# CrawlScript/tf_geometric

Measured on NVIDIA H100. Metric: edges/sec GCN+GAT fwd on 2.4M-node/123M-edge synthetic; %HBM roofline, higher is better.
Workload: dtype f32

## Files before the change

### include/tfgk.h

```cpp
#ifndef TFGK_H_
#define TFGK_H_

#include <stddef.h>
#include <stdint.h>

#ifdef __cplusplus
extern "C" {
#endif

#define TFGK_ABI_VERSION 7

enum tfgk_status {
    TFGK_OK = 0,
    TFGK_ERR_INVALID_ARGUMENT = 1,
    TFGK_ERR_CUDA = 2,
    TFGK_ERR_WORKSPACE = 3,
    TFGK_ERR_UNSUPPORTED = 4,
    TFGK_ERR_INDEX_OUT_OF_RANGE = 5
};

enum tfgk_reduce { TFGK_REDUCE_SUM = 0, TFGK_REDUCE_MEAN = 1, TFGK_REDUCE_MAX = 2 };
enum tfgk_act { TFGK_ACT_NONE = 0, TFGK_ACT_RELU = 1 };
enum tfgk_deg_power { TFGK_POW_INV_SQRT = 0, TFGK_POW_INV = 1 };
enum tfgk_heads_mode { TFGK_HEADS_SPLIT = 0, TFGK_HEADS_BROADCAST = 1, TFGK_HEADS_REDUCE = 2 };
// ... 50 lines not shown
int tfgk_permute_f32(const float *src, const int32_t *perm, int64_t E, int32_t width, float *dst, void *stream);
int tfgk_unpermute_f32(const float *src, const int32_t *perm, int64_t E, int32_t width, float *dst, void *stream);


int tfgk_csr_rowsum_f32(const int64_t *rowptr, const float *w_csr, int32_t N, float *out, void *stream);
int tfgk_deg_inv_f32(const float *deg, int32_t N, int power, float *out, void *stream);
int tfgk_scale_edges_f32(const int32_t *row, const int32_t *col, const float *w, int64_t E,
                         const float *dl, const float *dr, float *out, void *stream);


int tfgk_spmm_f32(const int64_t *rowptr, const int32_t *col, const float *w,
                  const float *h, int64_t ldh, int32_t n_dst, int32_t D, int reduce,
                  float alpha, const float *addend, int64_t ld_addend, float beta,
                  const float *bias, int act,
                  float *out, int64_t ldo, const tfgk_plan *plan, void *stream);
int tfgk_spmm_bf16(const int64_t *rowptr, const int32_t *col, const float *w,
                   const uint16_t *h, int64_t ldh, int32_t n_dst, int32_t D, int reduce,
                   float alpha, const float *addend, int64_t ld_addend, float beta,
                   const float *bias, int act,
                   float *out, int64_t ldo, const tfgk_plan *plan, void *stream);
int tfgk_spmm_bf16_dual(const int64_t *rowptr, const int32_t *col, const float *w,
                        const uint16_t *h, int64_t ldh, int32_t n_dst, int32_t D, int reduce,
                        float alpha, const float *addend, int64_t ld_addend, float beta,
                        const float *bias, int act,
                        float *out, int64_t ldo, uint16_t *out_bf16, int64_t ldob,
                        const tfgk_plan *plan, void *stream);

int tfgk_spmm_fp8(const int64_t *rowptr, const int32_t *col, const float *w,
                  const uint8_t *h, int64_t ldh, const int8_t *h_exp, int32_t n_dst, int32_t D, int reduce,
                  float alpha, const float *addend, int64_t ld_addend, float beta,
// ... 234 lines not shown
```

### tf_geometric_b200/_ffi.py

```python
import ctypes
import os
import threading

_LIB_PATH = os.path.join(os.path.dirname(os.path.abspath(__file__)), "lib", "libtfgk.so")
_lock = threading.Lock()
_lib = None

ABI_VERSION = 7

OK = 0
ERR_INVALID_ARGUMENT, ERR_CUDA, ERR_WORKSPACE, ERR_UNSUPPORTED, ERR_INDEX_OUT_OF_RANGE = 1, 2, 3, 4, 5
REDUCE_SUM, REDUCE_MEAN, REDUCE_MAX = 0, 1, 2
ACT_NONE, ACT_RELU = 0, 1
POW_INV_SQRT, POW_INV = 0, 1
HEADS_SPLIT, HEADS_BROADCAST, HEADS_REDUCE = 0, 1, 2
FLAG_ALL, FLAG_UPPER, FLAG_MAPPED = 0, 1, 2
BERNOULLI_NONE, BERNOULLI_DROPOUT, BERNOULLI_KEEP = 0, 1, 2
SAMPLE_NO_PADDING, SAMPLE_PADDING, SAMPLE_HEAD = 0, 1, 2
NEG_UPPER, NEG_START = 0, 1
PAD_ROW_MAJOR, PAD_STEP_MAJOR = 0, 1
SPGEMM_GRAD_LEFT, SPGEMM_GRAD_RIGHT = 0, 1
DTYPE_F32, DTYPE_BF16, DTYPE_FP8_E4M3 = 0, 1, 2

_i32, _i64, _f32, _int = ctypes.c_int32, ctypes.c_int64, ctypes.c_float, ctypes.c_int
# ... 11 lines not shown
    "tfgk_edge_unique_workspace_bytes": [_i64, _i32, ctypes.POINTER(_size)],
    "tfgk_edge_unique": [_ptr, _ptr, _i64, _i32, _ptr, _ptr, ctypes.POINTER(_i32), _ptr, _size, _ptr],
    "tfgk_directed_workspace_bytes": [_i64, ctypes.POINTER(_size)],
    "tfgk_directed_edges": [_ptr, _i64, _i64, _ptr, _i64, _ptr, ctypes.POINTER(_i32), _ptr, _size, _ptr],
    "tfgk_plan_capacity": [_i64, _i32, _i32, _i32, _i32, ctypes.POINTER(_i64), ctypes.POINTER(_i64)],
    "tfgk_plan_workspace_bytes": [_i32, ctypes.POINTER(_size)],
    "tfgk_plan_build": [_ptr, _i32, _i32, _i32, _i32, _ptr, _ptr, _ptr, _ptr, _ptr, _ptr, _ptr, _ptr, _i64, _i64,
                        ctypes.POINTER(_i32), _ptr, _size, _ptr],
    "tfgk_permute_f32": [_ptr, _ptr, _i64, _i32, _ptr, _ptr],
    "tfgk_unpermute_f32": [_ptr, _ptr, _i64, _i32, _ptr, _ptr],
    "tfgk_csr_rowsum_f32": [_ptr, _ptr, _i32, _ptr, _ptr],
    "tfgk_deg_inv_f32": [_ptr, _i32, _int, _ptr, _ptr],
    "tfgk_scale_edges_f32": [_ptr, _ptr, _ptr, _i64, _ptr, _ptr, _ptr, _ptr],
    "tfgk_spmm_f32": [_ptr, _ptr, _ptr, _ptr, _i64, _i32, _i32, _int, _f32, _ptr, _i64, _f32, _ptr, _int, _ptr, _i64,
                      _ptr, _ptr],
    "tfgk_spmm_bf16": [_ptr, _ptr, _ptr, _ptr, _i64, _i32, _i32, _int, _f32, _ptr, _i64, _f32, _ptr, _int, _ptr, _i64,
                       _ptr, _ptr],
    "tfgk_spmm_bf16_dual": [_ptr, _ptr, _ptr, _ptr, _i64, _i32, _i32, _int, _f32, _ptr, _i64, _f32, _ptr, _int, _ptr,
                            _i64, _ptr, _i64, _ptr, _ptr],
    "tfgk_spmm_fp8": [_ptr, _ptr, _ptr, _ptr, _i64, _ptr, _i32, _i32, _int, _f32, _ptr, _i64, _f32, _ptr, _int, _ptr,
                      _i64, _ptr, _ptr],
    "tfgk_segment_softmax_f32": [_ptr, _ptr, _i32, _i32, _ptr, _ptr],
    "tfgk_gat_fused_f32": [_ptr, _ptr, _ptr, _i64, _ptr, _i64, _ptr, _i64, _i32, _i32, _i32, _i32, _f32, _int, _ptr,
                           _int, _ptr, _int, _ptr, _i64, _ptr, _ptr],
    "tfgk_gat_fused_bf16": [_ptr, _ptr, _ptr, _i64, _ptr, _i64, _ptr, _i64, _i32, _i32, _i32, _i32, _f32, _int, _ptr,
                            _int, _ptr, _int, _ptr, _i64, _ptr, _ptr],
    "tfgk_gat_fused_fp8": [_ptr, _ptr, _ptr, _i64, _ptr, _i64, _ptr, _i32, _i32, _i32, _f32, _ptr, _int, _ptr, _i64, _ptr,
                           _ptr],
    "tfgk_gat_pack_keys_f32": [_ptr, _i64, _i32, _i32, _ptr, _i64, _ptr, _ptr],
    "tfgk_gat_fused_packed_f32": [_ptr, _ptr, _ptr, _i64, _ptr, _i64, _ptr, _i32, _i32, _i32, _f32, _ptr, _int, _ptr, _i64,
# ... 210 lines not shown
```

### tf_geometric_b200/csrc/spmm.cu

```cuda
#include "common.cuh"
#include <cuda_bf16.h>

namespace tfgk {

template <int VEC> struct Vec;
template <> struct Vec<4> { using T = float4; };
template <> struct Vec<1> { using T = float; };

template <int VEC>
__device__ __forceinline__ void load_vec(const float *p, float (&v)[VEC]) {
    if constexpr (VEC == 4) {
        const float4 t = __ldg(reinterpret_cast<const float4 *>(p));
        v[0] = t.x; v[1] = t.y; v[2] = t.z; v[3] = t.w;
    } else {
        v[0] = __ldg(p);
    }
}

template <int VEC>
__device__ __forceinline__ void load_vec(const uint16_t *p, float (&v)[VEC]) {
    static_assert(VEC == 1, "bf16 rows take the scalar path");
    v[0] = bf16_to_f32(__ldg(p));
}

// ... 32 lines not shown
    const float *bias;
    int act;
    float *out;
    int64_t ldo;
    uint16_t *outb;
    int64_t ldob;
    int32_t d_store;
    bool io4;
    int32_t n_tasks;
    const int32_t *task_row, *task_nrows;
    const int64_t *task_e0, *task_e1;
    const int32_t *task_slot;
    int32_t n_hubs;
    const int32_t *hub_row, *hub_slot0, *hub_nslots;
    float *scratch;
};

template <typename T> __device__ __forceinline__ const T *rows_of(const SpmmParams &p);
template <> __device__ __forceinline__ const float *rows_of<float>(const SpmmParams &p) { return p.h; }
template <> __device__ __forceinline__ const uint16_t *rows_of<uint16_t>(const SpmmParams &p) { return p.hb; }
template <> __device__ __forceinline__ const uint8_t *rows_of<uint8_t>(const SpmmParams &p) { return p.h8; }

template <int N>
__device__ __forceinline__ void epilogue_dual(const SpmmParams &p, int64_t r, int c, const float (&acc)[N], float cnt) {
    if (c >= p.d_store) return;
    float ad[N], bs[N], o[N];
    if constexpr (N == 4) {
        if (p.io4) {
            if (p.addend) load_vec<4>(p.addend + r * p.ld_addend + c, ad);
            if (p.bias) load_vec<4>(p.bias + c, bs);
// ... 316 lines not shown
        }
        if ((g + S) % RPC == 0) {
            const int dead = (g + S) / RPC - 1;
            if (dead & 1) load_chunk(dead + 2, cb, wnb); else load_chunk(dead + 2, ca, wna);
        }
    }
    if (slot >= 0) {
#pragma unroll
        for (int k = 0; k < NC; ++k)
            if (cok[k]) store_vec<4>(p.scratch + (int64_t)slot * p.D + coff[k], acc[k]);
        return;
    }
    while (r < r1) finalize_row();
}

__device__ __forceinline__ void tma_row(uint32_t dst, const void *src, uint32_t bytes, uint32_t bar) {
    asm volatile("cp.async.bulk.shared::cluster.global.mbarrier::complete_tx::bytes [%0], [%1], %2, [%3];"
                 ::"r"(dst), "l"(src), "r"(bytes), "r"(bar) : "memory");
}

__device__ __forceinline__ void mbar_wait_parity(uint32_t bar, uint32_t parity) {
    uint32_t done = 0;
    for (uint32_t spin = 0; !done; ++spin) {
        asm volatile(
            "{\n\t.reg .pred p;\n\t"
            "mbarrier.try_wait.parity.shared::cta.b64 p, [%1], %2;\n\t"
            "selp.u32 %0, 1, 0, p;\n\t}"
            : "=r"(done) : "r"(bar), "r"(parity) : "memory");
        if (spin > (1u << 28)) __trap();
    }
}

template <bool IS_MAX, int S, typename T, bool DUAL = false>
__global__ void __launch_bounds__(kAsyncWarps * 32) spmm_tma4_kernel(const SpmmParams p, uint32_t row_bytes) {
    constexpr int U = 4, RPC = 32 / U;
    constexpr bool FP8 = sizeof(T) == 1;
    static_assert(S <= 2 * RPC, "weight look-ahead registers would be overwritten before they are consumed");
    extern __shared__ __align__(128) uint8_t g4_ring[];
    const int lane = threadIdx.x & 31, warp = threadIdx.x >> 5;
    const uint32_t stage_bytes = (U * row_bytes + 127u) & ~127u;
    uint8_t *my_ring = g4_ring + (size_t)warp * S * stage_bytes;
    const uint32_t ring_addr = (uint32_t)__cvta_generic_to_shared(my_ring);
    uint64_t *bars = reinterpret_cast<uint64_t *>(g4_ring + (size_t)kAsyncWarps * S * stage_bytes) + warp * S;
    uint16_t *sexp = reinterpret_cast<uint16_t *>(g4_ring + (size_t)kAsyncWarps * S * (stage_bytes + 8)) + warp * S * U;
    const uint32_t bar0 = (uint32_t)__cvta_generic_to_shared(bars);
    if (lane == 0) {
#pragma unroll
        for (int i = 0; i < S; ++i) asm volatile("mbarrier.init.shared::cta.b64 [%0], 1;" ::"r"(bar0 + 8 * i));
        asm volatile("fence.mbarrier_init.release.cluster;" ::: "memory");
    }
    __syncwarp();
    const int64_t task = (int64_t)blockIdx.x * kAsyncWarps + warp;
    int64_t r0, r1, e_begin, e_stop;
    int slot = -1;
    if (p.task_row != nullptr) {
        if (task >= p.n_tasks) return;
        r0 = p.task_row[task];
        r1 = r0 + p.task_nrows[task];
        e_begin = p.task_e0[task];
        e_stop = p.task_e1[task];
        slot = p.task_slot[task];
    } else {
        r0 = task * kAsyncRows;
        if (r0 >= p.n_dst) return;
        r1 = min((int64_t)p.n_dst, r0 + kAsyncRows);
        e_begin = p.rowptr[r0];
        e_stop = p.rowptr[r1];
// ... 6 lines not shown
    constexpr int NCX = 2;
    int coff[NCX];
    bool cok[NCX];
    float acc[NCX][4];
#pragma unroll
    for (int k = 0; k < NCX; ++k) {
        coff[k] = (lane + 32 * k) * 4;
        cok[k] = coff[k] < p.D;
#pragma unroll
        for (int x = 0; x < 4; ++x) acc[k][x] = IS_MAX ? -FLT_MAX : 0.0f;
    }
    int64_t r = r0;
    int row_end = slot >= 0 ? 0x7fffffff : (int)(__shfl_sync(0xffffffffu, rp_hi, 0) - e_begin);
    const bool is_mean = p.reduce == TFGK_REDUCE_MEAN;

    auto finalize_row = [&]() {
        const int64_t row_start = __shfl_sync(0xffffffffu, rp_lo, (int)(r - r0));
        const int deg = (int)(row_end + e_begin - row_start);
        const float cnt = (float)max(deg, 1);
#pragma unroll
        for (int k = 0; k < NCX; ++k) {
            if (DUAL && cok[k]) {
                epilogue_dual<4>(p, r, coff[k], acc[k], cnt);
#pragma unroll
                for (int x = 0; x < 4; ++x) acc[k][x] = IS_MAX ? -FLT_MAX : 0.0f;
            } else if (cok[k]) {
                float ad[4], bs[4], o[4];
                if (p.addend) load_vec<4>(p.addend + r * p.ld_addend + coff[k], ad);
                if (p.bias) load_vec<4>(p.bias + coff[k], bs);
#pragma unroll
                for (int x = 0; x < 4; ++x) {
                    float a = acc[k][x];
                    if (is_mean) a = __fdiv_rn(a, cnt);
                    if (p.addend) a = __fadd_rn(__fmul_rn(a, p.alpha), __fmul_rn(ad[x], p.beta));
                    else if (p.alpha != 1.0f) a = __fmul_rn(a, p.alpha);
                    if (p.bias) a = __fadd_rn(a, bs[x]);
                    o[x] = apply_act(a, p.act);
                    acc[k][x] = IS_MAX ? -FLT_MAX : 0.0f;
                }
                store_vec<4>(p.out + r * p.ldo + coff[k], o);
            }
        }
        ++r;
        if (r < r1) row_end = (int)(__shfl_sync(0xffffffffu, rp_hi, (int)(r - r0)) - e_begin);
    };
    auto load_chunk = [&](int c, int &ci, float &wi) {
        const int e = c * 32 + lane;
        ci = 0;
        wi = 1.0f;
        if (e < n_edges) {
            ci = ld_stream_i32(p.col + e_begin + e);
            if (weighted) wi = ld_stream_f32(p.w + e_begin + e);
        }
    };
    uint32_t xpend = 0;
    int xslot = -1;
    auto issue = [&](int g, int ci) {
        if constexpr (FP8) {
// ... 69 lines not shown
        if ((g + 1) % RPC == 0) {
            if (cc & 1) wb = wnb; else wa = wna;
        }
        if ((g + S) % RPC == 0) {
            const int dead = (g + S) / RPC - 1;
            if (dead & 1) load_chunk(dead + 2, cb, wnb); else load_chunk(dead + 2, ca, wna);
        }
    }
    if (slot >= 0) {
#pragma unroll
        for (int k = 0; k < NCX; ++k)
            if (cok[k]) store_vec<4>(p.scratch + (int64_t)slot * p.D + coff[k], acc[k]);
        return;
    }
    while (r < r1) finalize_row();
}

template <bool IS_MAX, bool DUAL = false>
__global__ void __launch_bounds__(256) spmm_hub_fixup_kernel(const SpmmParams p) {
    const int lane = threadIdx.x & 31;
    const int h = blockIdx.x * 8 + (threadIdx.x >> 5);
    if (h >= p.n_hubs) return;
    const int64_t r = p.hub_row[h];
    const int s0 = p.hub_slot0[h], ns = p.hub_nslots[h];
    const float cnt = (float)max((int)(p.rowptr[r + 1] - p.rowptr[r]), 1);
    for (int c = lane * 4; c < p.D; c += 128) {
        float acc[4] = {IS_MAX ? -FLT_MAX : 0.f, IS_MAX ? -FLT_MAX : 0.f, IS_MAX ? -FLT_MAX : 0.f, IS_MAX ? -FLT_MAX : 0.f};
        for (int s = 0; s < ns; ++s) {
            float v[4];
            load_vec<4>(p.scratch + (int64_t)(s0 + s) * p.D + c, v);
#pragma unroll
            for (int x = 0; x < 4; ++x) acc[x] = IS_MAX ? fmaxf(acc[x], v[x]) : __fadd_rn(acc[x], v[x]);
        }
        if constexpr (DUAL) {
            epilogue_dual<4>(p, r, c, acc, cnt);
            continue;
        }
        float ad[4], bs[4], o[4];
        if (p.addend) load_vec<4>(p.addend + r * p.ld_addend + c, ad);
        if (p.bias) load_vec<4>(p.bias + c, bs);
#pragma unroll
        for (int x = 0; x < 4; ++x) {
            float a = acc[x];
            if (p.reduce == TFGK_REDUCE_MEAN) a = __fdiv_rn(a, cnt);
            if (p.addend) a = __fadd_rn(__fmul_rn(a, p.alpha), __fmul_rn(ad[x], p.beta));
            else if (p.alpha != 1.0f) a = __fmul_rn(a, p.alpha);
            if (p.bias) a = __fadd_rn(a, bs[x]);
            o[x] = apply_act(a, p.act);
        }
        store_vec<4>(p.out + r * p.ldo + c, o);
    }
}

template <int NC, int U, int S, typename T = float, bool DUAL = false>
static int launch_spmm_async(const SpmmParams &p, cudaStream_t st) {
    const uint32_t row_bytes = (uint32_t)(p.D * sizeof(T));
    const size_t smem = (size_t)kAsyncWarps * S * U * row_bytes;
    if (smem > 200 * 1024) return TFGK_ERR_UNSUPPORTED;
    const int64_t n_tasks = p.task_row ? p.n_tasks : ceil_div64(p.n_dst, kAsyncRows);
    const unsigned blocks = (unsigned)ceil_div64(n_tasks, kAsyncWarps);
    if (p.reduce == TFGK_REDUCE_MAX) {
        TFGK_CUDA(ensure_dynamic_smem(spmm_async_kernel<NC, true, U, S, T, DUAL>, smem));
        spmm_async_kernel<NC, true, U, S, T, DUAL><<<blocks, kAsyncWarps * 32, smem, st>>>(p, row_bytes);
    } else {
        TFGK_CUDA(ensure_dynamic_smem(spmm_async_kernel<NC, false, U, S, T, DUAL>, smem));
        spmm_async_kernel<NC, false, U, S, T, DUAL><<<blocks, kAsyncWarps * 32, smem, st>>>(p, row_bytes);
    }
    TFGK_LAUNCH_CHECK();
    if (p.task_row && p.n_hubs > 0) {
        const unsigned fb = (unsigned)ceil_div64(p.n_hubs, 8);
        if (p.reduce == TFGK_REDUCE_MAX) spmm_hub_fixup_kernel<true, DUAL><<<fb, 256, 0, st>>>(p);
        else spmm_hub_fixup_kernel<false, DUAL><<<fb, 256, 0, st>>>(p);
        TFGK_LAUNCH_CHECK();
    }
    return TFGK_OK;
}

template <int S, typename T = float, bool DUAL = false>
static int launch_spmm_tma4(const SpmmParams &p, cudaStream_t st) {
    constexpr int kPer16 = 16 / (int)sizeof(T);
    const void *base = sizeof(T) == 4 ? (const void *)p.h : sizeof(T) == 2 ? (const void *)p.hb : (const void *)p.h8;
    if (p.D > 256 || p.D % kPer16 != 0 || p.ldh % kPer16 != 0 || !aligned16(base)) return TFGK_ERR_UNSUPPORTED;
    const uint32_t row_bytes = (uint32_t)(p.D * sizeof(T));
    const size_t stage_pitch = ((size_t)4 * row_bytes + 127) & ~(size_t)127;
    const size_t smem = (size_t)kAsyncWarps * S * stage_pitch + (size_t)kAsyncWarps * S * 8 +
                        (sizeof(T) == 1 ? (size_t)kAsyncWarps * S * 4 * sizeof(uint16_t) : 0);
    if (smem > 200 * 1024) return TFGK_ERR_UNSUPPORTED;
    const int64_t n_tasks = p.task_row ? p.n_tasks : ceil_div64(p.n_dst, kAsyncRows);
    const unsigned blocks = (unsigned)ceil_div64(n_tasks, kAsyncWarps);
    if (p.reduce == TFGK_REDUCE_MAX) {
        TFGK_CUDA(ensure_dynamic_smem(spmm_tma4_kernel<true, S, T, DUAL>, smem));
        spmm_tma4_kernel<true, S, T, DUAL><<<blocks, kAsyncWarps * 32, smem, st>>>(p, row_bytes);
    } else {
        TFGK_CUDA(ensure_dynamic_smem(spmm_tma4_kernel<false, S, T, DUAL>, smem));
        spmm_tma4_kernel<false, S, T, DUAL><<<blocks, kAsyncWarps * 32, smem, st>>>(p, row_bytes);
    }
    TFGK_LAUNCH_CHECK();
    if (p.task_row && p.n_hubs > 0) {
        const unsigned fb = (unsigned)ceil_div64(p.n_hubs, 8);
        if (p.reduce == TFGK_REDUCE_MAX) spmm_hub_fixup_kernel<true, DUAL><<<fb, 256, 0, st>>>(p);
        else spmm_hub_fixup_kernel<false, DUAL><<<fb, 256, 0, st>>>(p);
        TFGK_LAUNCH_CHECK();
    }
    return TFGK_OK;
}

template <typename T, bool DUAL = false>
static int dispatch_spmm_async(const SpmmParams &p, cudaStream_t st) {
    const int lanes = (p.D + 3) / 4;
    return lanes <= 32 ? launch_spmm_async<1, 4, 3, T, DUAL>(p, st)
         : lanes <= 64 ? launch_spmm_async<2, 4, 4, T, DUAL>(p, st)
         : lanes <= 96 ? launch_spmm_async<3, 4, 3, T, DUAL>(p, st)
                       : launch_spmm_async<4, 2, 4, T, DUAL>(p, st);
}

// ... 43 lines not shown
                              int reduce, float alpha, const float *addend, int64_t ld_addend, float beta,
                              const float *bias, int act, float *out, int64_t ldo, int c0, int width) {
    SpmmParams p;
    p.rowptr = rowptr; p.col = col; p.w = w;
    p.h = nullptr; p.hb = nullptr; p.ldh = ldh; p.n_dst = n_dst;
    p.h8 = nullptr; p.hexp = nullptr; p.n_grp = 0; p.grp0 = 0;
    p.D = width;
    p.reduce = reduce; p.alpha = alpha;
    p.addend = addend ? addend + c0 : nullptr; p.ld_addend = ld_addend; p.beta = beta;
    p.bias = bias ? bias + c0 : nullptr; p.act = act;
    p.out = out ? out + c0 : nullptr; p.ldo = ldo;
    p.outb = nullptr; p.ldob = 0; p.d_store = width; p.io4 = false;
    p.n_tasks = 0; p.task_row = nullptr; p.task_nrows = nullptr; p.task_e0 = nullptr; p.task_e1 = nullptr;
    p.task_slot = nullptr; p.n_hubs = 0; p.hub_row = nullptr; p.hub_slot0 = nullptr; p.hub_nslots = nullptr;
    p.scratch = nullptr;
    return p;
}

}

using namespace tfgk;

extern "C" int tfgk_spmm_f32(const int64_t *rowptr, const int32_t *col, const float *w,
                             const float *h, int64_t ldh, int32_t n_dst, int32_t D, int reduce,
                             float alpha, const float *addend, int64_t ld_addend, float beta,
                             const float *bias, int act,
                             float *out, int64_t ldo, const tfgk_plan *plan, void *stream) {
    bool nothing_to_do = true;
    const int vrc = spmm_validate(rowptr, h, ldh, n_dst, D, reduce, addend, ld_addend, act, out, ldo, plan, &nothing_to_do);
    if (vrc != TFGK_OK || nothing_to_do) return vrc;
// ... 5 lines not shown
    for (int c0 = 0; c0 < D; c0 += cols_per_launch) {
        SpmmParams p = spmm_params(rowptr, col, w, ldh, n_dst, reduce, alpha, addend, ld_addend, beta, bias, act, out, ldo,
                                   c0, (D - c0 < cols_per_launch) ? D - c0 : cols_per_launch);
        p.h = h + c0;
        if (plan != nullptr && plan->n_tasks > 0 && vec4 && D >= 32 && D <= cols_per_launch) use_plan(p, plan);
        if (vec4 && p.D >= 32) {
            int rcr = launch_spmm_tma4<3>(p, as_stream(stream));
            if (rcr == TFGK_ERR_UNSUPPORTED) rcr = dispatch_spmm_async<float>(p, as_stream(stream));
            if (rcr != TFGK_ERR_UNSUPPORTED) { if (rcr != TFGK_OK) return rcr; continue; }
        }
        const int lanes = (p.D + vec - 1) / vec;
        const int rc = vec4 ? dispatch_spmm<4>(p, lanes, as_stream(stream)) : dispatch_spmm<1>(p, lanes, as_stream(stream));
        if (rc != TFGK_OK) return rc;
    }
    return TFGK_OK;
}

extern "C" int tfgk_spmm_bf16(const int64_t *rowptr, const int32_t *col, const float *w,
                              const uint16_t *h, int64_t ldh, int32_t n_dst, int32_t D, int reduce,
                              float alpha, const float *addend, int64_t ld_addend, float beta,
                              const float *bias, int act,
                              float *out, int64_t ldo, const tfgk_plan *plan, void *stream) {
    bool nothing_to_do = true;
    const int vrc = spmm_validate(rowptr, h, ldh, n_dst, D, reduce, addend, ld_addend, act, out, ldo, plan, &nothing_to_do);
    if (vrc != TFGK_OK || nothing_to_do) return vrc;

    const bool rows4 = (D % 4 == 0) && (ldh % 4 == 0) && aligned8(h) && (ldo % 4 == 0) && aligned16(out) &&
                       (!addend || ((ld_addend % 4 == 0) && aligned16(addend))) && (!bias || aligned16(bias));
    cudaStream_t st = as_stream(stream);
    if (rows4 && D >= 32 && D <= 512) {
// ... 107 lines not shown
```

### tf_geometric_b200/dist.py

```python
import os

import torch
import torch.distributed as dist

from . import ops
from .ops import CSR

ROW_ALIGN = 128


class RowPartition(object):

    def __init__(self, num_nodes, world_size, rank, align=1):
        self.num_nodes = int(num_nodes)
        self.world_size = int(world_size)
        self.rank = int(rank)
        self.block = (self.num_nodes + self.world_size - 1) // self.world_size
        if align > 1 and self.world_size > 1:
            self.block = (self.block + align - 1) // align * align
        self.lo = min(self.rank * self.block, self.num_nodes)
        self.hi = min(self.lo + self.block, self.num_nodes)
        self.n_local = self.hi - self.lo
        self.padded_nodes = self.block * self.world_size

# ... 291 lines not shown
        raise NotImplementedError("{}: the partitioned (multi-GPU) path is forward-only; call it under torch.no_grad() "
                                  "(or with layers created without trainable=True)".format(what))


def _unwrap(x_local, dev):
    if isinstance(x_local, SharedRows):
        return x_local.x, x_local
    return ops.as_device(x_local, torch.float32, device=dev), None


def gcn_partitioned(pg, x_local, kernel, bias=None, activation=None, renorm=True, improved=False):
    dev = pg.edge_index.device
    _forward_only("gcn_partitioned", x_local, kernel, bias)
    x_local, shared = _unwrap(x_local, dev)
    csr, value_csr = pg.gcn_normed(renorm=renorm, improved=improved)
    h_full = shared.find(kernel) if shared is not None and kernel is not None else None
    if h_full is None:
        if kernel is None:
            h_full = pg.all_gather_rows(x_local)
        else:
            h_full = pg.project_all_rows(x_local, [[(ops.as_device(kernel, torch.float32, device=dev), None, ops.ACT_NONE)]])[0]
    act_code, leftover = ops.activation_code(activation)
    out = ops.spmm(csr, value_csr, h_full, reduce="sum",
                   bias=None if bias is None else ops.as_device(bias, torch.float32, device=dev), act=act_code)
    return leftover(out) if leftover is not None else out


def gat_partitioned(pg, x_local, query_kernel, query_bias, query_activation, key_kernel, key_bias, key_activation,
                    kernel, bias=None, activation=None, num_heads=1):
    dev = pg.edge_index.device
    _forward_only("gat_partitioned", x_local, query_kernel, query_bias, key_kernel, key_bias, kernel, bias)
    x_local, shared = _unwrap(x_local, dev)
    f32 = lambda t: None if t is None else ops.as_device(t, torch.float32, device=dev)
    q_act, q_left = ops.activation_code(query_activation)
    k_act, k_left = ops.activation_code(key_activation)
    if q_left is not None or k_left is not None:
        raise NotImplementedError("partitioned GAT supports relu / None for the query and key activations")
    kv_full = shared.find(key_kernel, kernel) if shared is not None else None
    wq, wk, wv = f32(query_kernel), f32(key_kernel), f32(kernel)
# ... 314 lines not shown
```

### tf_geometric_b200/layers/conv/gcn.py

```python
import warnings

from ... import ops
from ...sparse import SparseMatrix
from ...nn.conv.gcn import gcn, gcn_build_cache_for_graph, gcn_build_cache_by_adj
from ...utils.graph_utils import compute_num_or_size_splits
from .._base import Layer


class GCN(Layer):

    def __init__(self, units, activation=None, use_kernel=True, use_bias=True,
                 norm="both", add_self_loop=True, sym=True, renorm=True, improved=False,
                 edge_drop_rate=0.0, num_splits=None, num_or_size_splits=None,
                 kernel_regularizer=None, bias_regularizer=None, *args, message_dtype=None, **kwargs):
        super().__init__(*args, **kwargs)
        ops.conv_message_dtype(message_dtype)
        self.message_dtype = message_dtype
        self.units = units
        self.activation = activation
        self.use_kernel = use_kernel
        self.use_bias = use_bias
        self.edge_drop_rate = edge_drop_rate
        self.kernel = None
        self.bias = None
# ... 22 lines not shown

    def build_cache_by_adj(self, sparse_adj, override=False, cache=None):
        return gcn_build_cache_by_adj(sparse_adj, self.norm, self.add_self_loop, self.sym, self.renorm, self.improved,
                                      override=override, cache=cache)

    def build_cache_for_graph(self, graph, override=False):
        gcn_build_cache_for_graph(graph, self.norm, self.add_self_loop, self.sym, self.renorm, self.improved,
                                  override=override)

    def cache_normed_edge(self, graph, override=False):
        warnings.warn("'GCN.cache_normed_edge(graph, override)' is deprecated, use "
                      "'GCN.build_cache_for_graph(graph, override)' instead", DeprecationWarning)
        return self.build_cache_for_graph(graph, override=override)

    def partitioned_projections(self):
        return [((id(self.kernel),), [(self.kernel, None, ops.ACT_NONE)])] if self.use_kernel else []

    def _call_partitioned(self, x_local, pg):
        from ... import dist as tdist
        if not (self.norm == "both" and self.add_self_loop and self.sym):
            raise NotImplementedError("partitioned GCN implements the default normalisation (norm='both', self loops, sym)")
        return tdist.gcn_partitioned(pg, x_local, self.kernel, self.bias, self.activation, renorm=self.renorm,
                                     improved=self.improved)

    def call(self, inputs, cache=None, split=True, training=None, mask=None):
        if hasattr(inputs[1], "part") and hasattr(inputs[1], "project_all_rows"):
            if ops.conv_message_dtype(self.message_dtype) is not None:
                raise NotImplementedError("message_dtype={} is not implemented for partitioned graphs".format(
                    str(ops.conv_message_dtype(self.message_dtype)).replace("torch.", "")))
            return self._call_partitioned(inputs[0], inputs[1])
        if isinstance(inputs[1], SparseMatrix):
# ... 13 lines not shown
```

### tf_geometric_b200/nn/conv/gcn.py

```python
import torch

from ... import ops, autograd
from ...sparse import SparseMatrix, as_sparse_features, project_features
from ..kernel.map_reduce import gcn_mapper

CACHE_KEY_GCN_NORMED_ADJ_TEMPLATE = "gcn_normed_adj_{}_{}_{}_{}_{}"


def compute_cache_key(norm, add_self_loop, sym, renorm, improved):
    return CACHE_KEY_GCN_NORMED_ADJ_TEMPLATE.format(norm, add_self_loop, sym, renorm, improved)


def gcn_norm_adj(sparse_adj, norm="both", add_self_loop=True, sym=True, renorm=True, improved=False, cache=None):
    if cache is not None:
        cache_key = compute_cache_key(norm, add_self_loop, sym, renorm, improved)
        cached = cache.get(cache_key, None)
        if cached is not None:
            if isinstance(cached, SparseMatrix):
                return cached
            return SparseMatrix(cached[0], cached[1], cached[2])

    w = sparse_adj.value
    normed, aux = _normalize(sparse_adj, norm, add_self_loop, sym, renorm, improved)
    if cache is not None:
# ... 85 lines not shown
        if kernel is None:
            raise ValueError("a sparse feature matrix needs a kernel (reference gcn.py:266-272)")
        if autograd.needs_grad(kernel, bias, x_sparse.value, normed.value):
            h = autograd.propagate(x_sparse, ops.as_device(kernel, torch.float32, device=dev))
            h = autograd.propagate(normed, h, bias, act_code)
            return leftover(h) if leftover is not None else h
        h = project_features(x_sparse, kernel)
        h = normed.matmul(h, num_or_size_splits=num_or_size_splits, bias=bias, act=act_code)
        return leftover(h) if leftover is not None else h
    x = ops.as_device(x, torch.float32, device=dev)
    if autograd.needs_grad(x, kernel, bias, normed.value):
        h = x if kernel is None else autograd.Dense.apply(x, ops.as_device(kernel, torch.float32, device=dev), None,
                                                         ops.ACT_NONE)
        h = autograd.propagate(normed, h, bias, act_code)
        return leftover(h) if leftover is not None else h
    h = x if kernel is None else ops.gemm(x, ops.as_device(kernel, torch.float32, device=dev))
    h = normed.matmul(h, num_or_size_splits=num_or_size_splits, bias=bias, act=act_code)
    if leftover is not None:
        h = leftover(h)
    return h


def _gcn_bf16(x, sparse_adj, kernel, bias, activation, norm, add_self_loop, sym, renorm, improved, edge_drop_rate,
              num_or_size_splits, training, cache):
    from .gat import project
    if as_sparse_features(x) is not None:
        raise NotImplementedError("message_dtype=bfloat16 takes a dense x")
    if training and edge_drop_rate > 0.0:
        raise NotImplementedError("message_dtype=bfloat16 is for inference: edge dropout is not applied in bf16")
    normed = gcn_norm_adj(sparse_adj, norm=norm, add_self_loop=add_self_loop, sym=sym, renorm=renorm,
                          improved=improved, cache=cache)
# ... 43 lines not shown
```

### tf_geometric_b200/ops.py

```python
import ctypes

import numpy as np
import torch

from . import _ffi, _rng
from ._ffi import (REDUCE_SUM, REDUCE_MEAN, REDUCE_MAX, ACT_NONE, ACT_RELU, POW_INV_SQRT, POW_INV,
                   HEADS_SPLIT, HEADS_BROADCAST, HEADS_REDUCE, FLAG_ALL, FLAG_UPPER, FLAG_MAPPED,
                   BERNOULLI_NONE, BERNOULLI_DROPOUT, BERNOULLI_KEEP, SAMPLE_NO_PADDING, SAMPLE_PADDING, SAMPLE_HEAD,
                   NEG_UPPER, NEG_START, PAD_ROW_MAJOR, PAD_STEP_MAJOR, SPGEMM_GRAD_LEFT, SPGEMM_GRAD_RIGHT)

_REDUCE_CODES = {"sum": REDUCE_SUM, "mean": REDUCE_MEAN, "max": REDUCE_MAX}


def _require_cuda():
    if not torch.cuda.is_available():
        raise RuntimeError("tf_geometric_b200 needs a CUDA device (H100 / sm_90a); there is no CPU fallback")


def default_device():
    _require_cuda()
    return torch.device("cuda", torch.cuda.current_device())


def as_device(x, dtype=None, device=None):
# ... 249 lines not shown
    if w_csr is not None:
        _check(w_csr, torch.float32, "w_csr")
    if bias is not None:
        _check(bias, torch.float32, "bias")
    code = _REDUCE_CODES[reduce] if isinstance(reduce, str) else reduce
    plan_struct = plan.struct(d8 if dual else D, h.device) if plan is not None else None
    plan_ref = ctypes.byref(plan_struct) if plan_struct is not None else None
    if dual:
        _ffi.call("tfgk_spmm_bf16_dual", _p(csr.rowptr), _p(csr.col if col is None else col), _p(w_csr), _p(h), ldh,
                  n_dst, D, code, float(alpha), _p(addend), lda, float(beta), _p(bias), act, _p(out), ldo, _p(out_bf16),
                  ldob, plan_ref, _stream(h))
        return out if out is not None else out_bf16
    _ffi.call("tfgk_spmm_bf16" if h.dtype == torch.bfloat16 else "tfgk_spmm_f32", _p(csr.rowptr),
              _p(csr.col if col is None else col), _p(w_csr), _p(h), ldh, n_dst, D,
              code, float(alpha), _p(addend), lda, float(beta), _p(bias), act, _p(out), ldo, plan_ref, _stream(h))
    return out


def spmm_max(csr, w_csr, h):
    if h.dtype != torch.float32 or not h.is_cuda:
        raise TypeError("spmm_max: h must be a float32 CUDA tensor")
    ldh = _row_major_2d(h, "h")
    n, D = csr.n_rows, h.shape[1]
    if w_csr is not None:
        _check(w_csr, torch.float32, "w_csr")
    out = torch.empty((n, D), dtype=torch.float32, device=h.device)
    cnt = torch.empty((n, D), dtype=torch.int32, device=h.device)
    plan = getattr(csr, "plan", None)
    plan_struct = plan.struct(2 * D, h.device) if plan is not None else None
    _ffi.call("tfgk_spmm_max_f32", _p(csr.rowptr), _p(csr.col), _p(w_csr), _p(h), ldh, n, D, _p(out), max(D, 1), _p(cnt),
# ... 890 lines not shown
```

Before: 3.892 billion.

## Fuse GCN projection into SpMM epilogue when input width is below output width

Adds a fused aggregate-then-project SpMM kernel: when F < U <= 128, the kernel first aggregates the narrower input features x over neighbours through the TMA ring, then multiplies batches of aggregated rows by W held in shared memory, adds bias and applies the activation. This swaps the separate GEMM plus SpMM over the wider projected features for a single pass that gathers only F-wide rows and never writes the projected intermediate. Hub rows get a matching fixup kernel that projects after aggregation. The costs are extra shared memory for W and the per-warp staging rows, fewer warps per block, and per-warp FMA work in the epilogue.

```diff
diff --git a/include/tfgk.h b/include/tfgk.h
--- a/include/tfgk.h
+++ b/include/tfgk.h
@@ -88,6 +88,9 @@
                   float alpha, const float *addend, int64_t ld_addend, float beta,
                   const float *bias, int act,
                   float *out, int64_t ldo, const tfgk_plan *plan, void *stream);
+int tfgk_spmm_proj_f32(const int64_t *rowptr, const int32_t *col, const float *w,
+                       const float *x, int64_t ldx, int32_t n_dst, int32_t F, const float *W, int32_t U,
+                       const float *bias, int act, float *out, int64_t ldo, const tfgk_plan *plan, void *stream);
 int tfgk_spmm_bf16(const int64_t *rowptr, const int32_t *col, const float *w,
                    const uint16_t *h, int64_t ldh, int32_t n_dst, int32_t D, int reduce,
                    float alpha, const float *addend, int64_t ld_addend, float beta,
diff --git a/tf_geometric_b200/_ffi.py b/tf_geometric_b200/_ffi.py
--- a/tf_geometric_b200/_ffi.py
+++ b/tf_geometric_b200/_ffi.py
@@ -49,6 +49,7 @@
     "tfgk_scale_edges_f32": [_ptr, _ptr, _ptr, _i64, _ptr, _ptr, _ptr, _ptr],
     "tfgk_spmm_f32": [_ptr, _ptr, _ptr, _ptr, _i64, _i32, _i32, _int, _f32, _ptr, _i64, _f32, _ptr, _int, _ptr, _i64,
                       _ptr, _ptr],
+    "tfgk_spmm_proj_f32": [_ptr, _ptr, _ptr, _ptr, _i64, _i32, _i32, _ptr, _i32, _ptr, _int, _ptr, _i64, _ptr, _ptr],
     "tfgk_spmm_bf16": [_ptr, _ptr, _ptr, _ptr, _i64, _i32, _i32, _int, _f32, _ptr, _i64, _f32, _ptr, _int, _ptr, _i64,
                        _ptr, _ptr],
     "tfgk_spmm_bf16_dual": [_ptr, _ptr, _ptr, _ptr, _i64, _i32, _i32, _int, _f32, _ptr, _i64, _f32, _ptr, _int, _ptr,
diff --git a/tf_geometric_b200/csrc/spmm.cu b/tf_geometric_b200/csrc/spmm.cu
--- a/tf_geometric_b200/csrc/spmm.cu
+++ b/tf_geometric_b200/csrc/spmm.cu
@@ -70,6 +70,9 @@
     int32_t n_hubs;
     const int32_t *hub_row, *hub_slot0, *hub_nslots;
     float *scratch;
+    const float *pw;
+    int32_t pu;
+    bool pio4;
 };
 
 template <typename T> __device__ __forceinline__ const T *rows_of(const SpmmParams &p);
@@ -416,6 +419,61 @@
     while (r < r1) finalize_row();
 }
 
+template <int NB, bool PADDED>
+__device__ __forceinline__ void project_rows(const SpmmParams &p, const float *__restrict__ Wm, int ldw,
+                                             const float *agg, int ldagg, int nrows, int F, int64_t row0, int lane) {
+    const int c = lane * 4;
+    if (c >= p.pu) return;
+    float o[NB][4];
+#pragma unroll
+    for (int b = 0; b < NB; ++b)
+#pragma unroll
+        for (int x = 0; x < 4; ++x) o[b][x] = 0.0f;
+    for (int k = 0; k < F; k += 4) {
+        float wk[4][4];
+#pragma unroll
+        for (int i = 0; i < 4; ++i) {
+            if constexpr (PADDED) {
+                const float4 t = *reinterpret_cast<const float4 *>(Wm + (k + i) * ldw + c);
+                wk[i][0] = t.x; wk[i][1] = t.y; wk[i][2] = t.z; wk[i][3] = t.w;
+            } else {
+#pragma unroll
+                for (int x = 0; x < 4; ++x) wk[i][x] = c + x < p.pu ? __ldg(Wm + (int64_t)(k + i) * ldw + c + x) : 0.0f;
+            }
+        }
+#pragma unroll
+        for (int b = 0; b < NB; ++b) {
+            const float4 a = *reinterpret_cast<const float4 *>(agg + b * ldagg + k);
+#pragma unroll
+            for (int x = 0; x < 4; ++x) {
+                o[b][x] = fmaf(a.x, wk[0][x], o[b][x]);
+                o[b][x] = fmaf(a.y, wk[1][x], o[b][x]);
+                o[b][x] = fmaf(a.z, wk[2][x], o[b][x]);
+                o[b][x] = fmaf(a.w, wk[3][x], o[b][x]);
+            }
+        }
+    }
+    float bs[4] = {0.f, 0.f, 0.f, 0.f};
+    if (p.bias) {
+        if (p.pio4) load_vec<4>(p.bias + c, bs);
+        else
+#pragma unroll
+            for (int x = 0; x < 4; ++x) if (c + x < p.pu) bs[x] = p.bias[c + x];
+    }
+#pragma unroll
+    for (int b = 0; b < NB; ++b) {
+        if (b >= nrows) break;
+        float v[4];
+#pragma unroll
+        for (int x = 0; x < 4; ++x) v[x] = apply_act(p.bias ? __fadd_rn(o[b][x], bs[x]) : o[b][x], p.act);
+        float *dst = p.out + (row0 + b) * p.ldo + c;
+        if (p.pio4) store_vec<4>(dst, v);
+        else
+#pragma unroll
+            for (int x = 0; x < 4; ++x) if (c + x < p.pu) dst[x] = v[x];
+    }
+}
+
 __device__ __forceinline__ void tma_row(uint32_t dst, const void *src, uint32_t bytes, uint32_t bar) {
     asm volatile("cp.async.bulk.shared::cluster.global.mbarrier::complete_tx::bytes [%0], [%1], %2, [%3];"
                  ::"r"(dst), "l"(src), "r"(bytes), "r"(bar) : "memory");
@@ -433,26 +491,50 @@
     }
 }
 
-template <bool IS_MAX, int S, typename T, bool DUAL = false>
-__global__ void __launch_bounds__(kAsyncWarps * 32) spmm_tma4_kernel(const SpmmParams p, uint32_t row_bytes) {
+constexpr int kProjRows = 4;
+constexpr int kProjWarps = 8;
+
+template <bool PROJ, typename T>
+__host__ __device__ inline size_t tma4_smem_bytes(int warps, int S, uint32_t row_bytes, int D, int pu) {
+    const size_t stage_pitch = ((size_t)4 * row_bytes + 127) & ~(size_t)127;
+    size_t bytes = (size_t)warps * S * stage_pitch + (size_t)warps * S * 8 +
+                   (sizeof(T) == 1 ? (size_t)warps * S * 4 * sizeof(uint16_t) : 0);
+    if (PROJ) bytes = (bytes + 15) / 16 * 16 + ((size_t)D * ((pu + 3) / 4 * 4) + (size_t)warps * kProjRows * D) * 4;
+    return bytes;
+}
+
+template <bool IS_MAX, int S, typename T, bool DUAL, bool PROJ, int WARPS>
+__device__ __forceinline__ void spmm_tma4_body(const SpmmParams &p, uint32_t row_bytes) {
     constexpr int U = 4, RPC = 32 / U;
     constexpr bool FP8 = sizeof(T) == 1;
     static_assert(S <= 2 * RPC, "weight look-ahead registers would be overwritten before they are consumed");
+    static_assert(!PROJ || (!IS_MAX && !DUAL && sizeof(T) == 4), "the projection epilogue follows an fp32 sum");
     extern __shared__ __align__(128) uint8_t g4_ring[];
     const int lane = threadIdx.x & 31, warp = threadIdx.x >> 5;
     const uint32_t stage_bytes = (U * row_bytes + 127u) & ~127u;
     uint8_t *my_ring = g4_ring + (size_t)warp * S * stage_bytes;
     const uint32_t ring_addr = (uint32_t)__cvta_generic_to_shared(my_ring);
-    uint64_t *bars = reinterpret_cast<uint64_t *>(g4_ring + (size_t)kAsyncWarps * S * stage_bytes) + warp * S;
-    uint16_t *sexp = reinterpret_cast<uint16_t *>(g4_ring + (size_t)kAsyncWarps * S * (stage_bytes + 8)) + warp * S * U;
+    uint64_t *bars = reinterpret_cast<uint64_t *>(g4_ring + (size_t)WARPS * S * stage_bytes) + warp * S;
+    uint16_t *sexp = reinterpret_cast<uint16_t *>(g4_ring + (size_t)WARPS * S * (stage_bytes + 8)) + warp * S * U;
     const uint32_t bar0 = (uint32_t)__cvta_generic_to_shared(bars);
+    float *w_s = nullptr, *agg_s = nullptr;
+    const int ldw = (p.pu + 3) & ~3;
+    if constexpr (PROJ) {
+        w_s = reinterpret_cast<float *>(g4_ring + ((size_t)WARPS * S * (stage_bytes + 8) + 15) / 16 * 16);
+        agg_s = w_s + (size_t)p.D * ldw + (size_t)warp * kProjRows * p.D;
+        for (int i = threadIdx.x; i < p.D * ldw; i += WARPS * 32) {
+            const int k = i / ldw, c = i - k * ldw;
+            w_s[i] = c < p.pu ? __ldg(p.pw + (int64_t)k * p.pu + c) : 0.0f;
+        }
+        __syncthreads();
+    }
     if (lane == 0) {
 #pragma unroll
         for (int i = 0; i < S; ++i) asm volatile("mbarrier.init.shared::cta.b64 [%0], 1;" ::"r"(bar0 + 8 * i));
         asm volatile("fence.mbarrier_init.release.cluster;" ::: "memory");
     }
     __syncwarp();
-    const int64_t task = (int64_t)blockIdx.x * kAsyncWarps + warp;
+    const int64_t task = (int64_t)blockIdx.x * WARPS + warp;
     int64_t r0, r1, e_begin, e_stop;
     int slot = -1;
     if (p.task_row != nullptr) {
@@ -489,13 +571,25 @@
     int row_end = slot >= 0 ? 0x7fffffff : (int)(__shfl_sync(0xffffffffu, rp_hi, 0) - e_begin);
     const bool is_mean = p.reduce == TFGK_REDUCE_MEAN;
 
+    int n_done = 0;
+    auto project_done = [&]() {
+        __syncwarp();
+        project_rows<kProjRows, true>(p, w_s, ldw, agg_s, p.D, n_done, p.D, r - n_done, lane);
+        __syncwarp();
+        n_done = 0;
+    };
     auto finalize_row = [&]() {
         const int64_t row_start = __shfl_sync(0xffffffffu, rp_lo, (int)(r - r0));
         const int deg = (int)(row_end + e_begin - row_start);
         const float cnt = (float)max(deg, 1);
 #pragma unroll
         for (int k = 0; k < NCX; ++k) {
-            if (DUAL && cok[k]) {
+            if (PROJ) {
+                if (k == 0 && cok[0])
+                    *reinterpret_cast<float4 *>(agg_s + n_done * p.D + coff[0]) = make_float4(acc[0][0], acc[0][1], acc[0][2], acc[0][3]);
+#pragma unroll
+                for (int x = 0; x < 4; ++x) acc[k][x] = 0.0f;
+            } else if (DUAL && cok[k]) {
                 epilogue_dual<4>(p, r, coff[k], acc[k], cnt);
 #pragma unroll
                 for (int x = 0; x < 4; ++x) acc[k][x] = IS_MAX ? -FLT_MAX : 0.0f;
@@ -517,6 +611,9 @@
             }
         }
         ++r;
+        if constexpr (PROJ) {
+            if (++n_done == kProjRows) project_done();
+        }
         if (r < r1) row_end = (int)(__shfl_sync(0xffffffffu, rp_hi, (int)(r - r0)) - e_begin);
     };
     auto load_chunk = [&](int c, int &ci, float &wi) {
@@ -616,10 +713,23 @@
         return;
     }
     while (r < r1) finalize_row();
-}
-
-template <bool IS_MAX, bool DUAL = false>
-__global__ void __launch_bounds__(256) spmm_hub_fixup_kernel(const SpmmParams p) {
+    if constexpr (PROJ) {
+        if (n_done > 0) project_done();
+    }
+}
+
+template <bool IS_MAX, int S, typename T, bool DUAL = false>
+__global__ void __launch_bounds__(kAsyncWarps * 32) spmm_tma4_kernel(const SpmmParams p, uint32_t row_bytes) {
+    spmm_tma4_body<IS_MAX, S, T, DUAL, false, kAsyncWarps>(p, row_bytes);
+}
+
+template <int S, int WARPS>
+__global__ void __launch_bounds__(WARPS * 32) spmm_proj_tma4_kernel(const SpmmParams p, uint32_t row_bytes) {
+    spmm_tma4_body<false, S, float, false, true, WARPS>(p, row_bytes);
+}
+
+template <bool IS_MAX, bool DUAL, bool PROJ>
+__device__ __forceinline__ void spmm_hub_fixup_body(const SpmmParams &p, float (*agg_s)[128]) {
     const int lane = threadIdx.x & 31;
     const int h = blockIdx.x * 8 + (threadIdx.x >> 5);
     if (h >= p.n_hubs) return;
@@ -634,6 +744,10 @@
 #pragma unroll
             for (int x = 0; x < 4; ++x) acc[x] = IS_MAX ? fmaxf(acc[x], v[x]) : __fadd_rn(acc[x], v[x]);
         }
+        if constexpr (PROJ) {
+            store_vec<4>(&agg_s[threadIdx.x >> 5][c], acc);
+            continue;
+        }
         if constexpr (DUAL) {
             epilogue_dual<4>(p, r, c, acc, cnt);
             continue;
@@ -652,6 +766,20 @@
         }
         store_vec<4>(p.out + r * p.ldo + c, o);
     }
+    if constexpr (PROJ) {
+        __syncwarp();
+        project_rows<1, false>(p, p.pw, p.pu, agg_s[threadIdx.x >> 5], 128, 1, p.D, r, lane);
+    }
+}
+
+template <bool IS_MAX, bool DUAL = false>
+__global__ void __launch_bounds__(256) spmm_hub_fixup_kernel(const SpmmParams p) {
+    spmm_hub_fixup_body<IS_MAX, DUAL, false>(p, nullptr);
+}
+
+__global__ void __launch_bounds__(256) spmm_hub_fixup_proj_kernel(const SpmmParams p) {
+    __shared__ __align__(16) float agg_s[8][128];
+    spmm_hub_fixup_body<false, false, true>(p, agg_s);
 }
 
 template <int NC, int U, int S, typename T = float, bool DUAL = false>
@@ -678,19 +806,20 @@
     return TFGK_OK;
 }
 
-template <int S, typename T = float, bool DUAL = false>
+template <int S, typename T = float, bool DUAL = false, bool PROJ = false, int WARPS = kAsyncWarps>
 static int launch_spmm_tma4(const SpmmParams &p, cudaStream_t st) {
     constexpr int kPer16 = 16 / (int)sizeof(T);
     const void *base = sizeof(T) == 4 ? (const void *)p.h : sizeof(T) == 2 ? (const void *)p.hb : (const void *)p.h8;
     if (p.D > 256 || p.D % kPer16 != 0 || p.ldh % kPer16 != 0 || !aligned16(base)) return TFGK_ERR_UNSUPPORTED;
     const uint32_t row_bytes = (uint32_t)(p.D * sizeof(T));
-    const size_t stage_pitch = ((size_t)4 * row_bytes + 127) & ~(size_t)127;
-    const size_t smem = (size_t)kAsyncWarps * S * stage_pitch + (size_t)kAsyncWarps * S * 8 +
-                        (sizeof(T) == 1 ? (size_t)kAsyncWarps * S * 4 * sizeof(uint16_t) : 0);
+    const size_t smem = tma4_smem_bytes<PROJ, T>(WARPS, S, row_bytes, p.D, PROJ ? p.pu : 0);
     if (smem > 200 * 1024) return TFGK_ERR_UNSUPPORTED;
     const int64_t n_tasks = p.task_row ? p.n_tasks : ceil_div64(p.n_dst, kAsyncRows);
-    const unsigned blocks = (unsigned)ceil_div64(n_tasks, kAsyncWarps);
-    if (p.reduce == TFGK_REDUCE_MAX) {
+    const unsigned blocks = (unsigned)ceil_div64(n_tasks, WARPS);
+    if constexpr (PROJ) {
+        TFGK_CUDA(ensure_dynamic_smem(spmm_proj_tma4_kernel<S, WARPS>, smem));
+        spmm_proj_tma4_kernel<S, WARPS><<<blocks, WARPS * 32, smem, st>>>(p, row_bytes);
+    } else if (p.reduce == TFGK_REDUCE_MAX) {
         TFGK_CUDA(ensure_dynamic_smem(spmm_tma4_kernel<true, S, T, DUAL>, smem));
         spmm_tma4_kernel<true, S, T, DUAL><<<blocks, kAsyncWarps * 32, smem, st>>>(p, row_bytes);
     } else {
@@ -700,7 +829,8 @@
     TFGK_LAUNCH_CHECK();
     if (p.task_row && p.n_hubs > 0) {
         const unsigned fb = (unsigned)ceil_div64(p.n_hubs, 8);
-        if (p.reduce == TFGK_REDUCE_MAX) spmm_hub_fixup_kernel<true, DUAL><<<fb, 256, 0, st>>>(p);
+        if (PROJ) spmm_hub_fixup_proj_kernel<<<fb, 256, 0, st>>>(p);
+        else if (p.reduce == TFGK_REDUCE_MAX) spmm_hub_fixup_kernel<true, DUAL><<<fb, 256, 0, st>>>(p);
         else spmm_hub_fixup_kernel<false, DUAL><<<fb, 256, 0, st>>>(p);
         TFGK_LAUNCH_CHECK();
     }
@@ -774,6 +904,7 @@
     p.n_tasks = 0; p.task_row = nullptr; p.task_nrows = nullptr; p.task_e0 = nullptr; p.task_e1 = nullptr;
     p.task_slot = nullptr; p.n_hubs = 0; p.hub_row = nullptr; p.hub_slot0 = nullptr; p.hub_nslots = nullptr;
     p.scratch = nullptr;
+    p.pw = nullptr; p.pu = 0; p.pio4 = false;
     return p;
 }
 
@@ -809,6 +940,27 @@
         if (rc != TFGK_OK) return rc;
     }
     return TFGK_OK;
+}
+
+extern "C" int tfgk_spmm_proj_f32(const int64_t *rowptr, const int32_t *col, const float *w,
+                                  const float *x, int64_t ldx, int32_t n_dst, int32_t F, const float *W, int32_t U,
+                                  const float *bias, int act, float *out, int64_t ldo, const tfgk_plan *plan, void *stream) {
+    TFGK_CHECK_ARG(n_dst >= 0 && F >= 0 && U >= 0, "spmm_proj: negative size (n_dst=%d, F=%d, U=%d)", n_dst, F, U);
+    TFGK_CHECK_ARG(act == TFGK_ACT_NONE || act == TFGK_ACT_RELU, "spmm_proj: unknown activation %d", act);
+    if (F < 4 || F % 4 != 0 || F >= U || U > 128 || ldx % 4 != 0 || !aligned16(x)) return TFGK_ERR_UNSUPPORTED;
+    TFGK_CHECK_ARG(ldx >= F && ldo >= U, "spmm_proj: leading dimension too small (ldx=%lld, ldo=%lld)", (long long)ldx,
+                   (long long)ldo);
+    if (plan != nullptr && plan->n_hubs > 0 && F >= 32)
+        TFGK_CHECK_ARG(plan->scratch != nullptr && plan->scratch_bytes >= (size_t)plan->n_slots * F * sizeof(float),
+                       "spmm_proj: plan scratch too small (need %zu bytes)", (size_t)plan->n_slots * F * sizeof(float));
+    if (n_dst == 0) return TFGK_OK;
+    TFGK_CHECK_ARG(rowptr && x && W && out, "spmm_proj: null pointer");
+    SpmmParams p = spmm_params(rowptr, col, w, ldx, n_dst, TFGK_REDUCE_SUM, 1.0f, nullptr, 0, 0.0f, bias, act, out, ldo, 0, F);
+    p.h = x;
+    p.pw = W; p.pu = U;
+    p.pio4 = U % 4 == 0 && ldo % 4 == 0 && aligned16(out) && (!bias || aligned16(bias));
+    if (plan != nullptr && plan->n_tasks > 0 && F >= 32) use_plan(p, plan);
+    return launch_spmm_tma4<3, float, false, true, kProjWarps>(p, as_stream(stream));
 }
 
 extern "C" int tfgk_spmm_bf16(const int64_t *rowptr, const int32_t *col, const float *w,
diff --git a/tf_geometric_b200/dist.py b/tf_geometric_b200/dist.py
--- a/tf_geometric_b200/dist.py
+++ b/tf_geometric_b200/dist.py
@@ -329,15 +329,19 @@
     _forward_only("gcn_partitioned", x_local, kernel, bias)
     x_local, shared = _unwrap(x_local, dev)
     csr, value_csr = pg.gcn_normed(renorm=renorm, improved=improved)
+    act_code, leftover = ops.activation_code(activation)
+    bias = None if bias is None else ops.as_device(bias, torch.float32, device=dev)
+    if kernel is not None and x_local.is_cuda and ops.spmm_proj_shape(x_local.shape[1], kernel.shape[1]):
+        out = ops.spmm_proj(csr, value_csr, pg.all_gather_rows(x_local),
+                            ops.as_device(kernel, torch.float32, device=dev), bias=bias, act=act_code)
+        return leftover(out) if leftover is not None else out
     h_full = shared.find(kernel) if shared is not None and kernel is not None else None
     if h_full is None:
         if kernel is None:
             h_full = pg.all_gather_rows(x_local)
         else:
             h_full = pg.project_all_rows(x_local, [[(ops.as_device(kernel, torch.float32, device=dev), None, ops.ACT_NONE)]])[0]
-    act_code, leftover = ops.activation_code(activation)
-    out = ops.spmm(csr, value_csr, h_full, reduce="sum",
-                   bias=None if bias is None else ops.as_device(bias, torch.float32, device=dev), act=act_code)
+    out = ops.spmm(csr, value_csr, h_full, reduce="sum", bias=bias, act=act_code)
     return leftover(out) if leftover is not None else out
 
 
diff --git a/tf_geometric_b200/layers/conv/gcn.py b/tf_geometric_b200/layers/conv/gcn.py
--- a/tf_geometric_b200/layers/conv/gcn.py
+++ b/tf_geometric_b200/layers/conv/gcn.py
@@ -60,7 +60,9 @@
         return self.build_cache_for_graph(graph, override=override)
 
     def partitioned_projections(self):
-        return [((id(self.kernel),), [(self.kernel, None, ops.ACT_NONE)])] if self.use_kernel else []
+        if not self.use_kernel or (self.kernel.is_cuda and ops.spmm_proj_shape(self.kernel.shape[0], self.kernel.shape[1])):
+            return []
+        return [((id(self.kernel),), [(self.kernel, None, ops.ACT_NONE)])]
 
     def _call_partitioned(self, x_local, pg):
         from ... import dist as tdist
diff --git a/tf_geometric_b200/nn/conv/gcn.py b/tf_geometric_b200/nn/conv/gcn.py
--- a/tf_geometric_b200/nn/conv/gcn.py
+++ b/tf_geometric_b200/nn/conv/gcn.py
@@ -123,7 +123,12 @@
                                                          ops.ACT_NONE)
         h = autograd.propagate(normed, h, bias, act_code)
         return leftover(h) if leftover is not None else h
-    h = x if kernel is None else ops.gemm(x, ops.as_device(kernel, torch.float32, device=dev))
+    if kernel is not None:
+        kernel = ops.as_device(kernel, torch.float32, device=dev)
+        if num_or_size_splits is None and ops.spmm_proj_supported(x, kernel):
+            h = ops.spmm_proj(normed.csr, normed.value_csr, x, kernel, bias=bias, act=act_code)
+            return leftover(h) if leftover is not None else h
+    h = x if kernel is None else ops.gemm(x, kernel)
     h = normed.matmul(h, num_or_size_splits=num_or_size_splits, bias=bias, act=act_code)
     if leftover is not None:
         h = leftover(h)
diff --git a/tf_geometric_b200/ops.py b/tf_geometric_b200/ops.py
--- a/tf_geometric_b200/ops.py
+++ b/tf_geometric_b200/ops.py
@@ -287,6 +287,40 @@
     _ffi.call("tfgk_spmm_bf16" if h.dtype == torch.bfloat16 else "tfgk_spmm_f32", _p(csr.rowptr),
               _p(csr.col if col is None else col), _p(w_csr), _p(h), ldh, n_dst, D,
               code, float(alpha), _p(addend), lda, float(beta), _p(bias), act, _p(out), ldo, plan_ref, _stream(h))
+    return out
+
+
+def spmm_proj_supported(x, W):
+    if not (x.is_cuda and x.dtype == torch.float32 and x.dim() == 2 and W.dim() == 2):
+        return False
+    if W.shape[0] != x.shape[1] or not spmm_proj_shape(x.shape[1], W.shape[1]) or x.stride(1) != 1:
+        return False
+    return _row_major_2d(x, "x") % 4 == 0 and x.data_ptr() % 16 == 0
+
+
+def spmm_proj_shape(F, U):
+    return 4 <= F < U <= 128 and F % 4 == 0
+
+
+def spmm_proj(csr, w_csr, x, W, bias=None, act=ACT_NONE, out=None):
+    if not spmm_proj_supported(x, W):
+        raise ValueError("spmm_proj: unsupported x {} / W {} (fp32 CUDA, 4 <= F < U <= 128, F % 4 == 0, aligned rows)".format(
+            tuple(x.shape), tuple(W.shape)))
+    W = W.to(torch.float32).contiguous()
+    n_dst, F, U = csr.n_rows, x.shape[1], W.shape[1]
+    if out is None:
+        out = torch.empty((n_dst, U), dtype=torch.float32, device=x.device)
+    elif not (out.is_cuda and out.dtype == torch.float32 and tuple(out.shape) == (n_dst, U)):
+        raise TypeError("spmm_proj: out must be a float32 CUDA tensor of shape {}".format((n_dst, U)))
+    if w_csr is not None:
+        _check(w_csr, torch.float32, "w_csr")
+    if bias is not None:
+        _check(bias, torch.float32, "bias")
+    plan = getattr(csr, "plan", None)
+    plan_struct = plan.struct(F, x.device) if plan is not None else None
+    _ffi.call("tfgk_spmm_proj_f32", _p(csr.rowptr), _p(csr.col), _p(w_csr), _p(x), _row_major_2d(x, "x"), n_dst, F, _p(W),
+              U, _p(bias), act, _p(out), _row_major_2d(out, "out"),
+              ctypes.byref(plan_struct) if plan_struct is not None else None, _stream(x))
     return out
 
 
```

Result: faster. 4.032 billion (median of 6 runs) (+3.6%).
